# apapiu/transformer_latent_diffusion

Measured on AMD Instinct MI355X. Metric: images/sec (256px, 35-step CFG sampling), denoiser only, higher is better.
Workload: dtype bf16; 1 GPU; C1: 100M-param denoiser (d=768, L=12), 32x32x4 latents, 35 steps + CFG 6, DPM-Solver++(2M), 64 images/GPU (model batch 128); images_per_gpu=64, global_batch=64, n_iter=35, parallelism=single GPU

## Files before the change

### transformer_latent_diffusion_amd/csrc/tld_engine.hip

```cpp
#include "../../include/tld_hip.h"
#include "tld_common.h"
#include "tld_host.h"
#include "tld_refresh.h"
#include "tld_tail_fold_math.h"

#include <cmath>
#include <cstdarg>
#include <cstdio>
#include <cstring>
#include <cstdlib>
#include <map>
#include <string>
#include <unordered_map>
#include <vector>

using namespace tld;

namespace {
thread_local char g_err[512] = "";
}
namespace tld {
void set_last_error(const char* msg) { snprintf(g_err, sizeof(g_err), "%s", msg); }
thread_local uint64_t* g_path_sink = nullptr;
}
// ... 267 lines not shown
    launch_linear_f32(e->c_sin, e->ne, e->ff1_w, e->ff1_b, e->c_h1, e->d, Tn, e->ne, e->d, 1, s);
    launch_linear_f32(e->c_h1, e->d, e->ff3_w, e->ff3_b, e->c_pre, e->d, Tn, e->d, e->d, 0, s);
}

void cond_label_rows(tld_engine* e, int row0, int Tl, hipStream_t s) {
    launch_linear_f32(e->c_label, e->text, e->label_w, e->label_b, e->c_pre + (size_t)row0 * e->d, e->d, Tl,
                      e->text, e->d, 0, s);
}

int run_body(tld_engine* e, const float* x_src, int src_batch, int batch, const int* noise_row,
             const int* label_row, float* out, hipStream_t s, bool share_l0 = false, const int* src_row = nullptr) {
    const int d = e->d, M = batch * e->ntok;
    share_l0 = share_l0 && e->share_l0 && (src_row ? batch > src_batch && batch <= 2 * src_batch : batch == 2 * src_batch);
    if (int rc = debug_poison(e, s)) return rc;
    const int b0 = share_l0 ? src_batch : batch;
    resid_t* xe = share_l0 ? e->x_half : e->x;
    const bool fold1 = e->fold_ln1;
    const int ln_slots = gemm_resid_stat_slots(d);
    {
        ProfScope ps(e, KC_EMBED, s);
        EmbedParams ep{};
        ep.x = x_src; ep.conv_w = e->conv_w; ep.conv_b = e->conv_b; ep.ln1_w = e->pln1_w; ep.ln1_b = e->pln1_b;
        ep.lin_wt = e->plin_wt; ep.lin_w_hl = e->plin_w_hl; ep.lin_b = e->plin_b; ep.ln2_w = e->pln2_w; ep.ln2_b = e->pln2_b; ep.pos = e->pos;
        ep.tok = xe; ep.stats_out = fold1 ? e->ln_stats : nullptr; ep.batch = b0; ep.src_batch = src_batch; ep.C = e->cfg.n_channels;
        ep.src_row = share_l0 ? nullptr : src_row;
        ep.S = e->cfg.image_size; ep.p = e->cfg.patch_size; ep.grid = e->grid; ep.pd = e->pd; ep.d = d;
        ep.ntok = e->ntok;
        launch_embed(ep, s);
    }
    const int rdt = sizeof(resid_t) == 2 ? ST_BF16 : ST_F32;
    SNAP("tokens0", xe, rdt, s, (int64_t)b0 * e->ntok, d);
    for (int l = 0; l < e->L; ++l) {
        const Layer& Ly = e->layers[l];
        const bool half = share_l0 && l == 0;
        const int bl = half ? b0 : batch, Ml = bl * e->ntok;
        const bool fuse8 = e->fp8 && e->fp8_fused;
        SNAP(blk_name(l, "x_in"), half ? xe : e->x, rdt, s, Ml, d);
        if (fold1) SNAP(blk_name(l, "ln1"), e->ln_stats, ST_F32, s, Ml, kLnSlots, 2);
        if (!fold1) {
            ProfScope ps(e, KC_LN, s);
            if (fuse8 && layernorm_mx8_supported(d)) launch_layernorm_mx8(half ? xe : e->x, Ly.n1_w, Ly.n1_b, e->a8, e->as8, Ml, d, s);
            else { launch_layernorm_bf16(half ? xe : e->x, Ly.n1_w, Ly.n1_b, e->xn, Ml, d, s); SNAP(blk_name(l, "xn1"), e->xn, ST_BF16, s, Ml, d); }
        }
        const bool fused_qa = eng_fused_qa(e);
        if (fused_qa) {
            ProfScope ps(e, KC_GEMM_QKV, s);
            GemmParams g{};
            const bool pair = eng_qkv_pair(e, bl);
            g.A = half ? xe : e->x; g.lda = d; g.W = pair ? Ly.qkv_wp2 : Ly.qkv_wp; g.ldw = d; g.M = Ml; g.N = 3 * d; g.K = d;
            g.out_bf16 = e->att; g.ldo = d; g.ntok = e->ntok; g.d = d;
            g.ln_stats = e->ln_stats; g.ln_slots = l == 0 ? 2 : ln_slots; g.ln_c1 = pair ? Ly.qkv_c1p2 : Ly.qkv_c1p; g.ln_b1 = pair ? Ly.qkv_b1p2 : Ly.qkv_b1p;
            g.park = pair ? e->pair_park : nullptr;
            GEMM_TRY(blk_name(l, "QKV + attention"), launch_gemm(g, pair ? EPI_QKV_ATTN2 : EPI_QKV_ATTN, s));
        } else {
            ProfScope ps(e, KC_GEMM_QKV, s);
            GemmParams g{};
            g.A = e->xn; g.lda = d; g.W = Ly.qkv_w; g.ldw = d; g.M = Ml; g.N = 3 * d; g.K = d;
            g.out_bf16 = e->qk; g.ldo = 2 * d; g.vt = e->vt; g.ntok = e->ntok; g.d = d;
            if (e->fp8) {
                if (!(fuse8 && layernorm_mx8_supported(d))) launch_quant_mx8(e->xn, e->a8, e->as8, Ml, d, s);
                SNAP(blk_name(l, "a8_qkv.q"), e->a8, ST_U8, s, Ml, d); SNAP(blk_name(l, "a8_qkv.s"), e->as8, ST_MX8S, s, Ml, d / 32);
                g.f8 = 1; g.A = reinterpret_cast<const bf16*>(e->a8); g.W = reinterpret_cast<const bf16*>(Ly.qkv_w8);
                g.a_scale = e->as8; g.w_scale = Ly.qkv_s8;
            }
#ifdef TLD_RESID_BF16
            if (fold1) {
                g.A = half ? xe : e->x; g.W = Ly.qkv_wf; g.ln_stats = e->ln_stats; g.ln_slots = l == 0 ? 2 : ln_slots;
                g.ln_c1 = Ly.qkv_c1; g.ln_b1 = Ly.qkv_b1;
            }
#endif
            GEMM_TRY(blk_name(l, "QKV projection"), launch_gemm(g, fold1 ? EPI_QKV_LN : EPI_QKV, s));
            SNAP(blk_name(l, "qk"), e->qk, ST_BF16, s, Ml, 2 * d); SNAP(blk_name(l, "vt"), e->vt, ST_BF16, s, bl, d, e->ntok);
        }
        if (!fused_qa) {
            ProfScope ps(e, KC_ATTN, s);
            launch_attention(e->qk, e->vt, e->att, bl, e->ntok, e->H, s);
        }
        SNAP(blk_name(l, "att"), e->att, ST_BF16, s, Ml, d);
        const bool fuse_dw = eng_fuse_dw(e);
        const bool fold3 = e->fold_ln3;
        {
            ProfScope ps(e, KC_CROSS, s);
            CrossRowParams cp{};
            cp.x = e->x; cp.att = e->att;
            cp.x_in = half ? xe : nullptr; cp.src_batch = src_batch; cp.src_row = src_row;
            cp.wq = e->c_wq + (size_t)l * e->cond_cap * e->H * d;
            cp.bwq = e->c_bwq + (size_t)l * e->cond_cap * e->H;
            cp.v = e->c_kv + (size_t)l * e->cond_cap * 2 * d + d;
            cp.v_ld = 2 * d;
            cp.noise_row = noise_row; cp.label_row = label_row;
            cp.ln2_w = Ly.n2_w; cp.ln2_b = Ly.n2_b; cp.ln3_w = Ly.n3_w; cp.ln3_b = Ly.n3_b;
            cp.xn3 = fold3 ? nullptr : e->xn; cp.ln3_stats = fold3 ? e->row_stats : nullptr; cp.batch = batch; cp.ntok = e->ntok; cp.d = d; cp.heads = e->H;
            if (e->dbg_keep) { if (int rc = e->stages.sink(blk_name(l, "sa"), M, d, &cp.sa_out)) return rc; }
            const bool cross8 = fuse8 && cross_row_supports_ln3_stats(d);
            if (cross8) { cp.xn3_f8 = e->a8; cp.xn3_s8 = e->as8; }
            launch_cross_row(cp, s);
            if (!fold3 && !cross8) SNAP(blk_name(l, "xn3"), e->xn, ST_BF16, s, M, d);
        }
        SNAP(blk_name(l, "ca"), e->x, rdt, s, M, d);
        if (fold3) SNAP(blk_name(l, "stats"), e->row_stats, ST_F32, s, M, 2);
        if (fuse_dw) {
            ProfScope ps(e, KC_GEMM_UP, s);
            GemmParams g{};
            g.A = e->xn; g.lda = d; g.W = Ly.up_w; g.ldw = d; g.M = M; g.N = e->hid; g.K = d;
            g.out_bf16 = e->hid2; g.ldo = e->hid; g.bias = Ly.up_b; g.dw_b = Ly.dw_b_half;
            g.dw_wpk = Ly.dw_wpk;
// ... 395 lines not shown
                if (pair_form) {
                    IMG(Ly.qkv_wp2, 3 * d * d) IMG(Ly.qkv_c1p2, 3 * d) IMG(Ly.qkv_b1p2, 3 * d)
                }
            }
        }
        if (e->fp8) {
            IMG(Ly.qkv_w8, 3 * d * d) IMG(Ly.qkv_s8, 3 * d * d / 32) IMG(Ly.up_w8, hid * d) IMG(Ly.up_s8, hid * d / 32)
            IMG(Ly.down_w8, d * hid) IMG(Ly.down_s8, d * hid / 32)
        }
        if (e->fold_ln3) { IMG(Ly.up_wf, hid * d) IMG(Ly.up_c1, hid) IMG(Ly.up_b1, hid) }
        IMG(Ly.dw_w9c, 9 * hid) IMG(Ly.dw_w9c_half, 9 * hid) IMG(Ly.dw_b_half, hid) IMG(Ly.dw_wpk, 12 * hid)
    }
    if (e->fold_tail && !e->fp8) {
        const size_t n = (size_t)(2 * tail_fold_padded_rows((int)pd) * (d + hid));
        IMG(e->out_fold_hl, n) IMG(e->out_fold_b, pd)
        HIP_TRY(hipMemsetAsync(e->out_fold_hl, 0, n * sizeof(bf16), nullptr));
        R.tail_fold_hl = e->out_fold_hl; R.tail_fold_b = e->out_fold_b;
    }
#undef IMG
    {
        const size_t L = (size_t)e->L;
        std::vector<const float*> tab(4 * L);
        for (size_t l = 0; l < L; ++l) { tab[l] = e->layers[l].kv_w; tab[L + l] = e->layers[l].q_w; tab[2 * L + l] = e->layers[l].n2_w; tab[3 * L + l] = e->layers[l].n2_b; }
        const float** tabs = nullptr;
        if (int rc = dev_alloc(e, &tabs, 4 * L)) return rc;
        e->tab_kv_w = tabs; e->tab_q_w = tabs + L; e->tab_n2_w = tabs + 2 * L; e->tab_n2_b = tabs + 3 * L;
        HIP_TRY(hipMemcpy(tabs, tab.data(), 4 * L * sizeof(float*), hipMemcpyHostToDevice));
        Layer* ld = nullptr;
        if (int rc = dev_alloc(e, &ld, L)) return rc;
        HIP_TRY(hipMemcpy(ld, e->layers.data(), L * sizeof(Layer), hipMemcpyHostToDevice));
        R.layers_dev = ld;
    }
    {
        struct Flat { float* p = nullptr; ~Flat() { if (p) (void)hipFree(p); } } flat;
        HIP_TRY(hipMalloc(&flat.p, (size_t)pl.count * sizeof(float)));
        for (const ParamTensor& q : pl.tensors)
            HIP_TRY(hipMemcpy(flat.p + q.off, e->host[q.key].data.data(), (size_t)q.numel * sizeof(float), hipMemcpyHostToDevice));
        e->host.clear();
        if (int rc = launch_refresh_weights(R, flat.p, nullptr)) return rc;
        HIP_TRY(hipStreamSynchronize(nullptr));
    }

    const size_t B2 = (size_t)e->cfg.max_batch, M = B2 * e->ntok;
    if (int rc = dev_alloc(e, &e->x, M * d)) return rc;
    if (int rc = dev_alloc(e, &e->x_half, M * d)) return rc;
    if (int rc = dev_alloc(e, &e->xn, M * d)) return rc;
    if (int rc = dev_alloc(e, &e->row_stats, M + 256)) return rc;
    if (int rc = dev_alloc(e, &e->ln_stats, (M + 256) * kLnSlots)) return rc;
    if (int rc = dev_alloc(e, &e->qk, M * 2 * d)) return rc;
    if (int rc = dev_alloc(e, &e->vt, M * d)) return rc;
    if (int rc = dev_alloc(e, &e->att, M * d)) return rc;
    if (pair_form) {
        const size_t pairs = B2 * (size_t)(e->H / 2), cus = (size_t)device_cu_count();
        if (int rc = dev_alloc(e, &e->pair_park, (pairs < cus ? pairs : cus) * (size_t)kPairSlotDwords)) return rc;
    }
    if (int rc = dev_alloc(e, &e->hid1, M * hid)) return rc;
    if (e->grid == 32 && e->fuse_dwconv && hid % 256 == 0) { if (int rc = dev_alloc(e, &e->seam, M * hid / 4)) return rc; }
    if (int rc = dev_alloc(e, &e->hid2, M * hid)) return rc;
    if (e->fp8) {
        if (int rc = dev_alloc(e, &e->a8, M * hid)) return rc;
        if (int rc = dev_alloc(e, &e->as8, M * hid / 32 + 1024)) return rc;
    }
    {
        auto& P = e->poison;
        P.clear();
        P.emplace_back(e->x, M * d * sizeof(resid_t)); P.emplace_back(e->x_half, M * d * sizeof(resid_t)); P.emplace_back(e->xn, M * d * 2);
        P.emplace_back(e->row_stats, (M + 256) * sizeof(float2)); P.emplace_back(e->ln_stats, (M + 256) * kLnSlots * sizeof(float2));
        P.emplace_back(e->qk, M * 2 * d * 2); P.emplace_back(e->vt, M * d * 2); P.emplace_back(e->att, M * d * 2);
        P.emplace_back(e->hid1, M * hid * 2); P.emplace_back(e->hid2, M * hid * 2);
        if (e->seam) P.emplace_back(e->seam, M * hid / 4 * sizeof(uint32_t));
    }
    if (int rc = dev_alloc(e, &e->io_x, B2 * e->img)) return rc;
    if (int rc = dev_alloc(e, &e->io_out, B2 * e->img)) return rc;
    if (int rc = dev_alloc(e, &e->io_sigma, B2)) return rc;
    if (int rc = dev_alloc(e, &e->io_label, B2 * e->text)) return rc;
    if (int rc = dev_alloc(e, &e->xt, B2 * e->img)) return rc;
    if (int rc = dev_alloc(e, &e->x0_prev, B2 * e->img)) return rc;
    if (int rc = ensure_cond_capacity(e, 2 * (int)B2)) return rc;
    if (int rc = dev_alloc(e, &e->rows_dev, 2 * B2)) return rc;
    if (int rc = ensure_req_capacity(e, 64 * (sizeof(SamplerStepRow) + 8 * B2))) return rc;
    e->finalized = true;
    return TLD_OK;
}

int64_t tld_engine_param_count(const tld_engine* e) { return e ? e->nparam : 0; }

int tld_engine_refresh_weights(tld_engine* e, const float* flat_device, int64_t numel, void* hip_stream) {
    if (!e || !flat_device) return fail(TLD_ERR_INVALID, "null argument");
    if (!e->finalized) return fail(TLD_ERR_STATE, "tld_engine_refresh_weights: weights not finalized (the first load goes through tld_engine_load_tensor)");
    if (numel != e->nparam)
        return fail(TLD_ERR_SHAPE, "tld_engine_refresh_weights: the flat vector has %lld elements, this configuration %lld", (long long)numel, (long long)e->nparam);
    DeviceGuard dg(e->cfg.device_id);
    return launch_refresh_weights(e->refresh, flat_device, static_cast<hipStream_t>(hip_stream));
}

int tld_engine_set_debug(tld_engine* e, int32_t enable) {
    if (!e) return fail(TLD_ERR_INVALID, "null engine");
    DeviceGuard dg(e->cfg.device_id);
    if (enable) {
        if (!e->finalized) return fail(TLD_ERR_STATE, "tld_engine_set_debug: weights not finalized");
        e->debug = true;
        if (int rc = reserve_snapshots(e)) { (void)hipDeviceSynchronize(); e->stages.free_all(); e->debug = false; return rc; }
    } else {
        (void)hipDeviceSynchronize();
        e->stages.free_all();
        e->debug = false; e->dbg_keep = false;
    }
// ... 504 lines not shown
```

### transformer_latent_diffusion_amd/csrc/tld_gemm.hip

```cpp
#include "../../include/tld_hip.h"
#include "tld_common.h"
#include "tld_attn_core.h"
#include <cstdlib>
#include <cstring>
#include <type_traits>

#ifdef TLD_DBG_EPI
#define TLD_EPI_BIT(b) ((p.dbg_epi & (b)) != 0)
#else
#define TLD_EPI_BIT(b) false
#endif

namespace tld {

namespace {

typedef const __attribute__((address_space(1))) void* gptr_t;
typedef __attribute__((address_space(3))) void* lptr_t;

__device__ __forceinline__ bf16x8 read_frag(const char* lds_tile, int row, int kchunk) {
    const int off = row * 128 + ((kchunk ^ ((row >> 1) & 7)) << 4);
    return *reinterpret_cast<const bf16x8*>(lds_tile + off);
}

template <int BN>
struct G256 {
    static constexpr int BM = 256, BK = 64;
    static constexpr int WN = (BN >= 256) ? 4 : 2, WMc = 8 / WN;
    static constexpr int WROWS = BM / WMc;
    static constexpr int WCOLS = BN / WN;
    static constexpr int TM = WROWS / 32, TN = WCOLS / 32;
    static constexpr int A_BYTES = BM * BK * 2, B_BYTES = BN * BK * 2;
    static constexpr int A_PIECES = BM / 8 / 8, B_PIECES = BN / 8 / 8;
};

template <int N> __device__ __forceinline__ void wait_vmcnt() {
    if constexpr (N == 0) asm volatile("s_waitcnt vmcnt(0)" ::: "memory");
    else if constexpr (N == 3) asm volatile("s_waitcnt vmcnt(3)" ::: "memory");
    else if constexpr (N == 4) asm volatile("s_waitcnt vmcnt(4)" ::: "memory");
    else if constexpr (N == 6) asm volatile("s_waitcnt vmcnt(6)" ::: "memory");
    else if constexpr (N == 7) asm volatile("s_waitcnt vmcnt(7)" ::: "memory");
    else if constexpr (N == 8) asm volatile("s_waitcnt vmcnt(8)" ::: "memory");
    else static_assert(N < 0, "unsupported vmcnt");
}

template <int BN>
struct G256P : G256<BN> {
    static constexpr int STAGES = 2;
    static constexpr int STAGE_BYTES = G256<BN>::A_BYTES + G256<BN>::B_BYTES;
    static constexpr int LDS_BYTES = 2 * STAGE_BYTES;
    static constexpr int LN_RAW = LDS_BYTES, LN_ST = LN_RAW + 256 * 8 * kLnSlots, LN_CB = LN_ST + 256 * 8, QKVLN_LDS = LN_CB + 2048;
    static constexpr int IMG2_PITCH = 1024, IMG2_BYTES = 128 * IMG2_PITCH;
    static constexpr int ZROW_OFF = IMG2_BYTES, ZROW_BYTES = 16 * IMG2_PITCH;
    static constexpr int ROWSTAT2_OFF = ZROW_OFF + ZROW_BYTES;
    static constexpr int CB2_OFF = ROWSTAT2_OFF + 256 * 8;
    static constexpr int UPDW2_LDS = CB2_OFF + 2048;
    static constexpr int PLAINRS_OFF = LDS_BYTES;
    static constexpr int PLAINCB_OFF = PLAINRS_OFF + 256 * 8;
    static constexpr int PLAINLN_LDS = PLAINCB_OFF + 2048;
    static constexpr int SCRATCH = 4608;
    static constexpr int AT_K = STAGE_BYTES, AT_V = AT_K + 256 * 128, AT_Q = AT_V + 64 * kAttnVPitch, ATTN_LDS = AT_Q + 256 * 128;
    static constexpr int P2_RAW = 0, P2_ST = P2_RAW + 256 * 8 * kLnSlots, P2_CB = P2_ST + 256 * 8;
    static constexpr int P2_K = P2_CB + 2 * 384 * 4 + 3072, P2_V = P2_K + 256 * 128, P2_Q = P2_V + 64 * kAttnVPitch, PAIR_LDS_END = P2_Q + 256 * 128;
};

template <int BN, int EPI, bool F8 = false, bool CONV = false, bool RING = false, bool TN = false>
__global__ __launch_bounds__(512) void gemm256p_kernel(GemmParams p, int nblocks) {
    using G = G256P<BN>;
    static_assert(!RING || BN == 256, "the half-tile ring exists for 256 x 256 tiles (bf16, and since round 6 MX-fp8)");
    static_assert(!TN || (BN == 256 && EPI == EPI_F32 && !F8 && !CONV && !RING), "transposed operands: fp32 output, 256 x 256 tiles, two-stage loop");
    using frag_t = std::conditional_t<F8, i32x8, bf16x8>;
    constexpr int ESZ = F8 ? 1 : 2;
    constexpr int SC_OFF = G::LDS_BYTES;
    static_assert(!F8 || (EPI == EPI_F32 || EPI == EPI_QKV || EPI == EPI_BIAS_BF16 || EPI == EPI_BIAS_RESID), "fp8 epilogues");
    static_assert(!CONV || (!F8 && (EPI == EPI_F32 || EPI == EPI_BIAS_BF16 || EPI == EPI_BIAS_RESID)), "conv mode");
    constexpr bool PLAIN_CB = EPI == EPI_BIAS_BF16 && BN != 384 && !F8 && !CONV;
    constexpr bool IS_QKV = EPI == EPI_QKV || EPI == EPI_QKV_LN, LN = EPI == EPI_QKV_LN || EPI == EPI_QKV_ATTN;
    constexpr bool UPDW = EPI == EPI_UP_DWCONV2 || EPI == EPI_UP_DWCONV32;
    static_assert(EPI != EPI_QKV_ATTN || (BN == 192 && !F8 && !CONV && !RING), "the fused attention epilogue is written for 256 x 192 tiles");
    static_assert(EPI != EPI_QKV_ATTN || G::ATTN_LDS <= 160 * 1024, "LDS");
    constexpr bool PAIR = EPI == EPI_QKV_ATTN2;
    static_assert(!PAIR || (BN == 384 && !F8 && !CONV && !RING && !TN), "the two-head attention epilogue is written for 256 x 384 tiles");
    static_assert(!PAIR || G::PAIR_LDS_END <= G::LDS_BYTES, "LDS");
    constexpr bool COLD = UPDW || PAIR;
    static_assert(8 * G::SCRATCH <= G::STAGE_BYTES, "epilogue scratch must fit in one stage");
    extern __shared__ __attribute__((aligned(16))) char smem[];
    const int lane = threadIdx.x & 63;
    const int wid = __builtin_amdgcn_readfirstlane(threadIdx.x >> 6);
    const int wm = wid / G::WN, wn = wid % G::WN;
    const int l31 = lane & 31, hi = lane >> 5;

    const int ntn = (p.N + BN - 1) / BN;
    const int ntm = (p.M + G::BM - 1) / G::BM;
    constexpr bool KSPLIT_OK = EPI == EPI_F32 && !F8 && !CONV && !RING && !TN;
    const int nsplit = (KSPLIT_OK && p.ksplit > 1) ? p.ksplit : 1;
    const int ntiles = ntm * ntn * nsplit;
    int kb_dec = 0;
    const int bid = blockIdx.x;
    const int xcd = bid & 7, lidx = bid >> 3;
    const int per_xcd_blocks = (nblocks + 7 - xcd) / 8;
    const int G2 = p.xcd_ngroups > 1 ? p.xcd_ngroups : 1;
    const int xn = xcd % G2, xm = xcd / G2, XM = 8 / G2;
    const int gcols = ntn / G2;
    const int r0 = (int)((long)ntm * xm / XM), r1 = (int)((long)ntm * (xm + 1) / XM);
    const int q = ntiles >> 3, rr = ntiles & 7;
    const int xbase = xcd < rr ? xcd * (q + 1) : rr * (q + 1) + (xcd - rr) * q;
    const int xcount = G2 > 1 ? (r1 - r0) * gcols : q + (xcd < rr ? 1 : 0);
    int my_tiles = lidx < xcount ? (xcount - lidx + per_xcd_blocks - 1) / per_xcd_blocks : 0;
    constexpr bool HT_OK = RING && !CONV && (EPI == EPI_F32 || EPI == EPI_QKV || EPI == EPI_QKV_LN || EPI == EPI_BIAS_BF16);
    const int ht_q = xcount / per_xcd_blocks, ht_R = xcount - ht_q * per_xcd_blocks;
    const bool ht = HT_OK && p.half_tail && G2 == 1 && ht_R > 0 && 2 * ht_R <= per_xcd_blocks;
    const int ht_qa = lidx >= ht_R ? 1 : 0;
    if (ht) my_tiles = ht_q + (lidx < 2 * ht_R ? 1 : 0);
    auto item_tile = [&](int i) {
        if (ht && i == ht_q) return ht_q * per_xcd_blocks + (lidx < ht_R ? lidx : lidx - ht_R);
        return lidx + i * per_xcd_blocks;
    };
    auto tile_coords = [&](int i, int& m0, int& n0) {
        const int t = item_tile(i);
        if (G2 > 1) {
            const int tm = t / gcols;
            m0 = (r0 + tm) * G::BM;
            n0 = (xn * gcols + (t - tm * gcols)) * BN;
        } else {
            int tile = xbase + t;
            if constexpr (KSPLIT_OK) {
                if (nsplit > 1) {
                    const int sp = tile / (ntm * ntn);
                    tile -= sp * (ntm * ntn);
                    kb_dec = sp * p.K * 2;
                }
            }
            const int tm = tile / ntn;
            m0 = tm * G::BM;
            n0 = (tile - tm * ntn) * BN;
        }
// ... 355 lines not shown
                    __builtin_amdgcn_global_load_lds((gptr_t)src, (lptr_t)(smem + G::P2_CB + (wid & 1) * 1536 + (wid >> 1) * 1024), 16, 0, 0);
                }
            }
            if constexpr (EPI == EPI_BIAS_BF16) {
                if (BN != 384 && p.row_stats && wid < 2) {
                    int r0s = m0 + wid * 128 + lane * 2;
                    r0s = r0s + 1 < p.M ? r0s : (p.M >= 2 ? p.M - 2 : 0);
                    const char* src = reinterpret_cast<const char*>(p.row_stats + r0s);
                    __builtin_amdgcn_global_load_lds((gptr_t)src, (lptr_t)(smem + G::PLAINRS_OFF + wid * 1024), 16, 0, 0);
                }
                if constexpr (PLAIN_CB) {
                    if (wid == 3 || (wid == 2 && p.row_stats)) {
                        int col = n0 + lane * 4;
                        col = col < p.N ? col : 0;
                        const float* src = (wid == 2 ? p.ln_c1 : p.bias) + col;
                        __builtin_amdgcn_global_load_lds((gptr_t)src, (lptr_t)(smem + G::PLAINCB_OFF + (wid - 2) * 1024), 16, 0, 0);
                    }
                }
            }
            if constexpr (UPDW) {
                constexpr int RS_OFF = G::ROWSTAT2_OFF;
                if (p.row_stats && wid < 2) {
                    const char* src = reinterpret_cast<const char*>(p.row_stats + m0) + wid * 1024 + lane * 16;
                    __builtin_amdgcn_global_load_lds((gptr_t)src, (lptr_t)(smem + RS_OFF + wid * 1024), 16, 0, 0);
                }
                if (wid == 3 || (wid == 2 && p.row_stats)) {
                    const float* src = (wid == 2 ? p.ln_c1 : p.bias) + n0 + lane * 4;
                    __builtin_amdgcn_global_load_lds((gptr_t)src, (lptr_t)(smem + G::CB2_OFF + (wid - 2) * 1024), 16, 0, 0);
                }
            }
        };
        auto kloop = [&](auto swp) {
            constexpr bool SW = decltype(swp)::value;
            auto mma = [&](const frag_t (&a)[G::TM], const frag_t (&b)[G::TN], auto slice) {
                constexpr int S2 = decltype(slice)::value * 2;
#pragma unroll
                for (int i = 0; i < G::TM; ++i)
#pragma unroll
                    for (int j = 0; j < G::TN; ++j) {
                        if constexpr (F8) {
                            if constexpr (SW) acc[i][j] = __builtin_amdgcn_mfma_scale_f32_32x32x64_f8f6f4(b[j], a[i], acc[i][j], 0, 0, S2, scb[j], S2, sca[i]);
                            else acc[i][j] = __builtin_amdgcn_mfma_scale_f32_32x32x64_f8f6f4(a[i], b[j], acc[i][j], 0, 0, S2, sca[i], S2, scb[j]);
                        } else {
                            if constexpr (SW) acc[i][j] = __builtin_amdgcn_mfma_f32_32x32x16_bf16(b[j], a[i], acc[i][j], 0, 0, 0);
                            else acc[i][j] = __builtin_amdgcn_mfma_f32_32x32x16_bf16(a[i], b[j], acc[i][j], 0, 0, 0);
                        }
                    }
            };
            constexpr int NP = G::A_PIECES + G::B_PIECES;
            {
            const int grp = wid >> 2;
            wait_vmcnt<0>();
            __builtin_amdgcn_s_barrier();
            if (grp) __builtin_amdgcn_s_barrier();
            for (int k = 0; k < nkt; ++k, ++g) {
                if (k == (PAIR ? nkt - 1 : nkt > 1 ? 1 : 0)) aux_dma();
                const char* st = smem + (g & 1) * G::STAGE_BYTES;
                char* nst = smem + ((g + 1) & 1) * G::STAGE_BYTES;
                const bool more = (k + 1 < nkt) || (has_next && !COLD);
                const int pkb = (k + 1 < nkt) ? (KSPLIT_OK ? kb0 : 0) + (k + 1) * G::BK * 2 : (KSPLIT_OK ? kbn : 0);
                if constexpr (CONV) {
                    if (k + 1 < nkt) {
                        if (++ccb == kpt) { ccb = 0; ++ctap; conv_tap(ctap); }
                    } else { ccb = 0; ctap = 0; }
                    conv_akb = ccb * (G::BK * 2);
                }
                if (k + 1 == nkt && more) set_offsets(m0n, n0n);
                constexpr int NI = F8 ? 2 : 4;
                constexpr int NDMA = (NI == 4) ? 2 : 1;
#pragma unroll
                for (int h = 0; h < NI; ++h) {
                    load_frags(st, h, a0, b0);
                    if constexpr (F8) {
                        if (h == 0) {
                            const char* sc = smem + SC_OFF + (g & 1) * 2048;
#pragma unroll
                            for (int i = 0; i < G::TM; ++i) sca[i] = *reinterpret_cast<const int*>(sc + (wm * G::WROWS + i * 32 + l31) * 4) >> (8 * hi);
#pragma unroll
                            for (int j = 0; j < G::TN; ++j) scb[j] = *reinterpret_cast<const int*>(sc + 1024 + (wn * G::WCOLS + j * 32 + l31) * 4) >> (8 * hi);
                        }
                    }
                    if (h < NDMA && more) {
                        constexpr int PER = (NP + NDMA - 1) / NDMA;
#pragma unroll
                        for (int q2 = 0; q2 < NP; ++q2) {
                            if (q2 < h * PER || q2 >= (h + 1) * PER) continue;
                            dma_piece(q2, pkb, nst);
                        }
                        if (h == 0) {
                            if (k + 1 < nkt) dma_scales(m0, n0, k + 1, (g + 1) & 1);
                            else dma_scales(m0n, n0n, 0, (g + 1) & 1);
                        }
                    }
                    if (h == NI - 1) wait_vmcnt<0>();
                    if (h == NI - 1) asm volatile("s_waitcnt lgkmcnt(0)" ::: "memory");
                    __builtin_amdgcn_sched_barrier(0);
                    __builtin_amdgcn_s_barrier();
                    __builtin_amdgcn_sched_barrier(0);
                    __builtin_amdgcn_s_setprio(1);
                    if constexpr (F8) {
                        if (h == 0) mma(a0, b0, std::integral_constant<int, 0>{}); else mma(a0, b0, std::integral_constant<int, 1>{});
                    } else {
                        mma(a0, b0, std::integral_constant<int, 0>{});
                    }
                    __builtin_amdgcn_s_setprio(0);
                    if (h == NI - 1) wait_vmcnt<0>();
// ... 113 lines not shown
                        auto cat = [](const piece_t& lo, const piece_t& hi4) {
                            return i32x8{(int)lo[0], (int)lo[1], (int)lo[2], (int)lo[3], (int)hi4[0], (int)hi4[1], (int)hi4[2], (int)hi4[3]};
                        };
                        __builtin_amdgcn_s_setprio(1);
#pragma unroll
                        for (int sl = 0; sl < 2; ++sl) {
                            const i32x8 bo = qb ? cat(fb1[2 * sl], fb1[2 * sl + 1]) : cat(fb0[2 * sl], fb0[2 * sl + 1]);
#pragma unroll
                            for (int ii = 0; ii < 2; ++ii) {
                                const i32x8 ao = cat(fa[ii][2 * sl], fa[ii][2 * sl + 1]);
                                const int sa = ii ? sa1 : sa0;
                                if (sl == 0) {
                                    if constexpr (SW) acc[qa * 2 + ii][qb] = __builtin_amdgcn_mfma_scale_f32_32x32x64_f8f6f4(bo, ao, acc[qa * 2 + ii][qb], 0, 0, 0, sb, 0, sa);
                                    else acc[qa * 2 + ii][qb] = __builtin_amdgcn_mfma_scale_f32_32x32x64_f8f6f4(ao, bo, acc[qa * 2 + ii][qb], 0, 0, 0, sa, 0, sb);
                                } else {
                                    if constexpr (SW) acc[qa * 2 + ii][qb] = __builtin_amdgcn_mfma_scale_f32_32x32x64_f8f6f4(bo, ao, acc[qa * 2 + ii][qb], 0, 0, 2, sb, 2, sa);
                                    else acc[qa * 2 + ii][qb] = __builtin_amdgcn_mfma_scale_f32_32x32x64_f8f6f4(ao, bo, acc[qa * 2 + ii][qb], 0, 0, 2, sa, 2, sb);
                                }
                            }
                        }
                        __builtin_amdgcn_s_setprio(0);
                    } else {
                    __builtin_amdgcn_s_setprio(1);
#pragma unroll
                    for (int ks = 0; ks < 4; ++ks)
#pragma unroll
                        for (int ii = 0; ii < 2; ++ii) {
                            const piece_t& bf = qb ? fb1[ks] : fb0[ks];
                            if constexpr (SW) acc[qa * 2 + ii][qb] = __builtin_amdgcn_mfma_f32_32x32x16_bf16(bf, fa[ii][ks], acc[qa * 2 + ii][qb], 0, 0, 0);
                            else acc[qa * 2 + ii][qb] = __builtin_amdgcn_mfma_f32_32x32x16_bf16(fa[ii][ks], bf, acc[qa * 2 + ii][qb], 0, 0, 0);
                        }
                    __builtin_amdgcn_s_setprio(0);
                    }
                    }
                    __builtin_amdgcn_sched_barrier(0);
                    __builtin_amdgcn_s_barrier();
                    __builtin_amdgcn_sched_barrier(0);
                };
                phase(std::integral_constant<int, 1>{}); phase(std::integral_constant<int, 2>{});
                phase(std::integral_constant<int, 3>{}); phase(std::integral_constant<int, 4>{});
                phase(std::integral_constant<int, 5>{}); phase(std::integral_constant<int, 6>{});
                phase(std::integral_constant<int, 7>{}); phase(std::integral_constant<int, 8>{});
            };
            for (int j = 0; j + 1 < nj; ++j) iter(j, std::false_type{});
            iter(nj - 1, std::true_type{});
            if (xt) wait_vmcnt<0>();
            if (!grp) __builtin_amdgcn_s_barrier();
            g += nk;
            }
        };
        if constexpr (RING) {
            if constexpr (swapped) kloop_ring(std::true_type{}); else kloop_ring(std::false_type{});
        } else {
            if constexpr (swapped) kloop(std::true_type{}); else kloop(std::false_type{});
        }

        const int row0 = m0 + wm * G::WROWS;
        const int col0 = n0 + wn * G::WCOLS;
        auto gn_combine = [&](const float2* red) {
            if constexpr (CONV) {
                asm volatile("s_waitcnt lgkmcnt(0)" ::: "memory");
                __builtin_amdgcn_s_barrier();
                const int tid = wid * 64 + lane;
                const int qpg = p.gn_cpg >> 2;
                if (tid < BN / p.gn_cpg) {
                    float a = 0.f, a2 = 0.f;
                    for (int w2 = 0; w2 < G::WMc; ++w2)
                        for (int k2 = 0; k2 < qpg; ++k2) { const float2 t = red[w2 * (BN / 4) + tid * qpg + k2]; a += t.x; a2 += t.y; }
                    const int bb = m0 / p.gn_hw;
                    const int chunk = (m0 - bb * p.gn_hw) >> 8, nchunk = p.gn_hw >> 8;
                    p.gn_partial[((size_t)bb * nchunk + chunk) * p.gn_groups + n0 / p.gn_cpg + tid] = make_float2(a, a2);
                }
            }
        };
        if constexpr (EPI == EPI_F32) {
#pragma unroll
            for (int i = 0; i < G::TM; ++i)
#pragma unroll
                for (int j = 0; j < G::TN; ++j) {
                    const int col = col0 + j * 32 + l31;
                    if (col >= p.N || (hmode && (i >> 1) != ht_qa)) continue;
#pragma unroll
                    for (int r = 0; r < 16; ++r) {
                        const int row = row0 + i * 32 + 4 * hi + (r & 3) + 8 * (r >> 2);
                        if (row < p.M) p.c_f32[(KSPLIT_OK && nsplit > 1 ? (size_t)(kb0 / (p.K * 2)) * p.M * p.ldc : (size_t)0) + (size_t)row * p.ldc + col] = acc[i][j][r];
                    }
                }
        } else {
            __builtin_amdgcn_s_barrier();
            char* ws = RING ? smem + 4 * HT + wid * G::SCRATCH : smem + ((g - 1) & 1) * G::STAGE_BYTES + wid * G::SCRATCH;
            if constexpr (UPDW) {
                static_assert(BN == 256, "fused depthwise epilogue is written for 256-column tiles");
                char* H = smem;
                {
                    if (it == 0) {
                        *reinterpret_cast<u32x4*>(smem + G::ZROW_OFF + threadIdx.x * 16) = u32x4{0u, 0u, 0u, 0u};
                        *reinterpret_cast<u32x4*>(smem + G::ZROW_OFF + 8192 + threadIdx.x * 16) = u32x4{0u, 0u, 0u, 0u};
                    }
                }
                const bool ln3 = p.row_stats != nullptr;
                float cst[G::TN], bst[G::TN];
#pragma unroll
                for (int j = 0; j < G::TN; ++j) {
                    const int cl = wn * 64 + j * 32 + l31;
                    bst[j] = *reinterpret_cast<const float*>(smem + G::CB2_OFF + 1024 + cl * 4);
                    cst[j] = ln3 ? *reinterpret_cast<const float*>(smem + G::CB2_OFF + cl * 4) : 0.f;
                }
// ... 365 lines not shown
#else
                    const float inv = attn256_wave(Kimg, Vimg, qf, o, e_l31, e_hi);
#endif
                    char* T = Qimg + wid * 4096;
                    bf16* dst0 = p.out_bf16 + (size_t)(m0 + q0) * p.ldo + (n0 / BN) * 64;
#pragma unroll
                    for (int half = 0; half < 2; ++half) {
                        if ((e_l31 >> 4) == half) {
#pragma unroll
                            for (int ct = 0; ct < 2; ++ct)
#pragma unroll
                                for (int rq = 0; rq < 4; ++rq) {
                                    bf16x4 pk;
#pragma unroll
                                    for (int e2 = 0; e2 < 4; ++e2) pk[e2] = (bf16)(o[ct][rq * 4 + e2] * inv);
                                    *reinterpret_cast<bf16x4*>(T + (e_l31 & 15) * 144 + ct * 64 + rq * 16 + e_hi * 8) = pk;
                                }
                        }
                        __builtin_amdgcn_fence(__ATOMIC_RELEASE, "wavefront");
#pragma unroll
                        for (int it2 = 0; it2 < 2; ++it2) {
                            const int r = it2 * 8 + (e_lane >> 3), c16 = e_lane & 7;
                            const u32x4 w = *reinterpret_cast<const u32x4*>(T + r * 144 + c16 * 16);
                            __builtin_nontemporal_store(w, reinterpret_cast<u32x4*>(dst0 + (size_t)(half * 16 + r) * p.ldo + c16 * 8));
                        }
                        __builtin_amdgcn_fence(__ATOMIC_ACQUIRE, "wavefront");
                    }
                }
            } else if constexpr (PAIR) {
                int e_lane = lane, e_l31 = l31, e_hi = hi;
                asm volatile("" : "+v"(e_lane), "+v"(e_l31), "+v"(e_hi));
                const int tid = wid * 64 + e_lane;
                {
                    const int s0 = (tid & 1) * 4;
                    const float4* raw = reinterpret_cast<const float4*>(smem + G::P2_RAW + (tid >> 1) * 64 + s0 * 8);
                    float su = 0.f, sq = 0.f;
#pragma unroll
                    for (int q2 = 0; q2 < 2; ++q2)
                        if (s0 + 2 * q2 < p.ln_slots) {
                            const float4 v = raw[q2];
                            su += v.x + v.z; sq += v.y + v.w;
                        }
                    su = dpp_add<0xB1>(su); sq = dpp_add<0xB1>(sq);
                    int kdim = p.K;
                    asm volatile("" : "+s"(kdim));
                    const float inv_k = 1.0f / (float)kdim;
                    const float mu = su * inv_k;
                    const float var = fmaxf(fmaf(sq, inv_k, -mu * mu), 0.f);
                    if (!(tid & 1))
                        reinterpret_cast<float2*>(smem + G::P2_ST)[tid >> 1] = make_float2(mu, __builtin_amdgcn_rsqf(var + kLnEps));
                    asm volatile("s_waitcnt lgkmcnt(0)" ::: "memory");
                    __builtin_amdgcn_s_barrier();
                }
                u32x4* slot = reinterpret_cast<u32x4*>(p.park) + (size_t)blockIdx.x * (kPairSlotDwords / 4) + tid;
                bf16x8 pk[G::TM][G::TN];
                {
                    float rs[G::TM], nm[G::TM];
#pragma unroll
                    for (int i = 0; i < G::TM; ++i) {
                        const float2 st = reinterpret_cast<const float2*>(smem + G::P2_ST)[wm * G::WROWS + i * 32 + e_l31];
                        rs[i] = st.y; nm[i] = -st.y * st.x;
                    }
#pragma unroll
                    for (int j = 0; j < G::TN; ++j) {
#pragma unroll
                        for (int rq = 0; rq < 4; ++rq) {
                            const int cl = wn * G::WCOLS + j * 32 + 8 * rq + 4 * e_hi;
                            const float4 c4 = *reinterpret_cast<const float4*>(smem + G::P2_CB + cl * 4);
                            const float4 b4 = *reinterpret_cast<const float4*>(smem + G::P2_CB + 1536 + cl * 4);
#pragma unroll
                            for (int i = 0; i < G::TM; ++i) {
                                acc[i][j][rq * 4 + 0] = fmaf(rs[i], acc[i][j][rq * 4 + 0], fmaf(nm[i], c4.x, b4.x));
                                acc[i][j][rq * 4 + 1] = fmaf(rs[i], acc[i][j][rq * 4 + 1], fmaf(nm[i], c4.y, b4.y));
                                acc[i][j][rq * 4 + 2] = fmaf(rs[i], acc[i][j][rq * 4 + 2], fmaf(nm[i], c4.z, b4.z));
                                acc[i][j][rq * 4 + 3] = fmaf(rs[i], acc[i][j][rq * 4 + 3], fmaf(nm[i], c4.w, b4.w));
                            }
                        }
#pragma unroll
                        for (int i = 0; i < G::TM; ++i) {
                            bf16x8 b;
#pragma unroll
                            for (int e2 = 0; e2 < 8; ++e2) b[e2] = (bf16)acc[i][j][8 + e2];
                            slot[(j * G::TM + i) * 512] = __builtin_bit_cast(u32x4, b);
                        }
                    }
#pragma unroll
                    for (int j = 0; j < G::TN; ++j)
#pragma unroll
                        for (int i = 0; i < G::TM; ++i)
#pragma unroll
                            for (int e2 = 0; e2 < 8; ++e2) pk[i][j][e2] = (bf16)acc[i][j][e2];
                }
                char* Kimg = smem + G::P2_K;
                char* Vimg = smem + G::P2_V;
                char* Qimg = smem + G::P2_Q;
                auto head = [&](int side) {
#pragma unroll
                    for (int j = 0; j < G::TN; ++j) {
#pragma unroll
                        for (int i = 0; i < G::TM; ++i) {
                            const int row = wm * G::WROWS + i * 32 + e_l31;
#pragma unroll
                            for (int rq = 0; rq < 2; ++rq) {
                                const bf16x4 q4 = {pk[i][j][rq * 4 + 0], pk[i][j][rq * 4 + 1], pk[i][j][rq * 4 + 2], pk[i][j][rq * 4 + 3]};
                                const int f = wn * 16 + 8 * rq + 4 * e_hi;
                                if (j < 2) {
                                    char* img = j == 0 ? Qimg : Kimg;
                                    *reinterpret_cast<bf16x4*>(img + row * 128 + ((((f >> 3) ^ ((row >> 1) & 7)) << 4) | ((f & 7) << 1))) = q4;
                                } else {
#pragma unroll
                                    for (int e2 = 0; e2 < 4; ++e2)
                                        *reinterpret_cast<bf16*>(Vimg + (f + e2) * kAttnVPitch + row * 2) = q4[e2];
                                }
                            }
                        }
                    }
                    asm volatile("s_waitcnt lgkmcnt(0)" ::: "memory");
                    __builtin_amdgcn_s_barrier();
                    const int q0 = wid * 32;
                    bf16x8 qf[4];
                    {
                        const int row = q0 + e_l31;
#pragma unroll
                        for (int ks = 0; ks < 4; ++ks)
                            qf[ks] = *reinterpret_cast<const bf16x8*>(Qimg + row * 128 + (((ks * 2 + e_hi) ^ ((row >> 1) & 7)) << 4));
                    }
                    f32x16 o[2];
                    const float inv = attn256_wave(Kimg, Vimg, qf, o, e_l31, e_hi);
                    char* T = Qimg + wid * 4096;
                    bf16* dst0 = p.out_bf16 + (size_t)(m0 + q0) * p.ldo + ((n0 / BN) * 2 + side) * 64;
#pragma unroll
                    for (int half = 0; half < 2; ++half) {
                        if ((e_l31 >> 4) == half) {
#pragma unroll
                            for (int ct = 0; ct < 2; ++ct)
#pragma unroll
                                for (int rq = 0; rq < 4; ++rq) {
                                    bf16x4 o4;
#pragma unroll
                                    for (int e2 = 0; e2 < 4; ++e2) o4[e2] = (bf16)(o[ct][rq * 4 + e2] * inv);
                                    *reinterpret_cast<bf16x4*>(T + (e_l31 & 15) * 144 + ct * 64 + rq * 16 + e_hi * 8) = o4;
                                }
                        }
                        __builtin_amdgcn_fence(__ATOMIC_RELEASE, "wavefront");
#pragma unroll
                        for (int it2 = 0; it2 < 2; ++it2) {
                            const int r = it2 * 8 + (e_lane >> 3), c16 = e_lane & 7;
                            const u32x4 w = *reinterpret_cast<const u32x4*>(T + r * 144 + c16 * 16);
                            __builtin_nontemporal_store(w, reinterpret_cast<u32x4*>(dst0 + (size_t)(half * 16 + r) * p.ldo + c16 * 8));
                        }
                        __builtin_amdgcn_fence(__ATOMIC_ACQUIRE, "wavefront");
                    }
                };
                head(0);
                wait_vmcnt<0>();
#pragma unroll
                for (int j = 0; j < G::TN; ++j)
#pragma unroll
                    for (int i = 0; i < G::TM; ++i) pk[i][j] = __builtin_bit_cast(bf16x8, slot[(j * G::TM + i) * 512]);
                __builtin_amdgcn_s_barrier();
                head(1);
                __builtin_amdgcn_s_barrier();
                if (has_next) issue(m0n, n0n, g);
            } else if constexpr (EPI == EPI_BIAS_BF16 && G::WCOLS == 96) {
                constexpr int P = 64 + 16;
                int e_lane = lane, e_l31 = l31, e_hi = hi;
                asm volatile("" : "+v"(e_lane), "+v"(e_l31), "+v"(e_hi));
#pragma unroll
                for (int i = 0; i < G::TM; ++i)
#pragma unroll
                    for (int j = 0; j < G::TN; ++j) {
#pragma unroll
                        for (int rq = 0; rq < 4; ++rq) {
                            const int cl = 8 * rq + 4 * e_hi;
                            const int cg = col0 + j * 32 + cl < p.N ? col0 + j * 32 + cl : 0;
                            const float4 bv = *reinterpret_cast<const float4*>(p.bias + cg);
                            bf16x4 pk;
                            pk[0] = (bf16)(acc[i][j][rq * 4 + 0] + bv.x); pk[1] = (bf16)(acc[i][j][rq * 4 + 1] + bv.y);
                            pk[2] = (bf16)(acc[i][j][rq * 4 + 2] + bv.z); pk[3] = (bf16)(acc[i][j][rq * 4 + 3] + bv.w);
                            *reinterpret_cast<bf16x4*>(ws + e_l31 * P + cl * 2) = pk;
                        }
#pragma unroll
                        for (int itr = 0; itr < 2; ++itr) {
                            const int idx = itr * 64 + e_lane;
                            const int rl = idx >> 2, ch = idx & 3;
                            const u32x4 v = *reinterpret_cast<const u32x4*>(ws + rl * P + ch * 16);
                            const int row = row0 + i * 32 + rl, col = col0 + j * 32 + ch * 8;
                            if (row < p.M && col < p.N) TLD_STORE(reinterpret_cast<u32x4*>(p.out_bf16 + (size_t)row * p.ldo + col), v);
                        }
                    }
            } else if constexpr (G::WCOLS == 64) {
                int e_lane = lane, e_l31 = l31, e_hi = hi;
                asm volatile("" : "+v"(e_lane), "+v"(e_l31), "+v"(e_hi));
                if constexpr (LN) {
                    {
                        const int tid = wid * 64 + e_lane;
                        const int s0 = (tid & 1) * 4;
                        const float4* raw = reinterpret_cast<const float4*>(smem + G::LN_RAW + (tid >> 1) * 64 + s0 * 8);
                        float su = 0.f, sq = 0.f;
#pragma unroll
                        for (int q2 = 0; q2 < 2; ++q2)
                            if (s0 + 2 * q2 < p.ln_slots) {
                                const float4 v = raw[q2];
                                su += v.x + v.z; sq += v.y + v.w;
                            }
                        su = dpp_add<0xB1>(su); sq = dpp_add<0xB1>(sq);
                        const float inv_k = 1.0f / (float)p.K;
                        const float mu = su * inv_k;
                        const float var = fmaxf(fmaf(sq, inv_k, -mu * mu), 0.f);
                        if (!(tid & 1))
                            reinterpret_cast<float2*>(smem + G::LN_ST)[tid >> 1] = make_float2(mu, __builtin_amdgcn_rsqf(var + kLnEps));
                        asm volatile("s_waitcnt lgkmcnt(0)" ::: "memory");
                        __builtin_amdgcn_s_barrier();
                    }
                    float rs[G::TM], nm[G::TM];
// ... 310 lines not shown
```

### transformer_latent_diffusion_amd/csrc/tld_gemm_params.h

```cpp
#pragma once
#include <stdint.h>
#ifndef __HIP__
struct float2;
#endif

namespace tld {

typedef __bf16 bf16;

#ifdef TLD_RESID_FP32
typedef float resid_t;
#else
#define TLD_RESID_BF16 1
typedef __bf16 resid_t;
#endif

constexpr int kLnSlots = 8;

enum GemmEpilogue {
    EPI_F32 = 0,
    EPI_QKV = 1,
    EPI_BIAS_BF16 = 2,
    EPI_BIAS_RESID = 3,
    EPI_QKV_LN = 5,
    EPI_UP_DWCONV32 = 4,
    EPI_UP_DWCONV2 = 6,
    EPI_QKV_ATTN = 7,
    EPI_QKV_ATTN2 = 9,
};

struct GemmParams {
    const bf16* A; int lda;
    const bf16* W; int ldw;
    int M, N, K;
    float* c_f32; int ldc;
    bf16* out_bf16; int ldo;
    bf16* vt;
    int ntok, d;
    const float* bias;
    const float* dw_b;
    uint32_t* dw_seam;
    const uint32_t* dw_wpk;
    resid_t* resid; int ldr;
    float2* stats_out;
    const float2* ln_stats;
    int ln_slots;
    const float* ln_b1;
    const float2* row_stats;
    const float* ln_c1;
    int f8;
    const uint8_t* a_scale;
    const uint8_t* w_scale;
    int w_batch_rows;
    unsigned w_batch_stride_bytes;
    int conv, cv_h, cv_w, cv_up, cv_cin;
    unsigned cv_data_off;
    float2* gn_partial;
    int gn_groups, gn_cpg, gn_hw;
    int ksplit;
    int xcd_ngroups;
    int tn_ktotal;
    int half_tail;
    int dbg_epi;
    int cv_down;
    uint32_t* park;
};

constexpr int kPairSlotDwords = 512 * 48;

}
```

Before: 317.5 images/s.

## Park half of the pair-attention QKV fragments in spare LDS instead of global memory

In the two-head fused QKV+attention epilogue, the second-half accumulator fragments were all parked in a per-block global scratch slot and reloaded after the first head. Six of the twelve entries now go into unused LDS regions around the pair layout, and the global slot shrinks to the other six. The global reloads are issued inside head 0, right after its output store, so they overlap with the remaining stores. The attention output staging also switches to a swizzled 32-row tile written in one pass instead of two 16-row halves. A compile-gated timestamp trace is added for profiling. The risk is more LDS pressure and possible layout conflicts, which the new static asserts are meant to catch.

```diff
diff --git a/transformer_latent_diffusion_amd/csrc/tld_engine.hip b/transformer_latent_diffusion_amd/csrc/tld_engine.hip
--- a/transformer_latent_diffusion_amd/csrc/tld_engine.hip
+++ b/transformer_latent_diffusion_amd/csrc/tld_engine.hip
@@ -343,6 +343,26 @@
             g.ln_stats = e->ln_stats; g.ln_slots = l == 0 ? 2 : ln_slots; g.ln_c1 = pair ? Ly.qkv_c1p2 : Ly.qkv_c1p; g.ln_b1 = pair ? Ly.qkv_b1p2 : Ly.qkv_b1p;
             g.park = pair ? e->pair_park : nullptr;
             GEMM_TRY(blk_name(l, "QKV + attention"), launch_gemm(g, pair ? EPI_QKV_ATTN2 : EPI_QKV_ATTN, s));
+#ifdef TLD_GEMM_TRACE_BUILD
+            if (pair) {
+                static int launches = 0;
+                static const char* path = getenv("TLD_GEMM_TRACE");
+                static const int at = getenv("TLD_GEMM_TRACE_LAUNCH") ? atoi(getenv("TLD_GEMM_TRACE_LAUNCH")) : 200;
+                if (path && ++launches == at) {
+                    std::vector<unsigned long long> st(kPairTraceDwords / 2);
+                    HIP_TRY(hipStreamSynchronize(s));
+                    HIP_TRY(hipMemcpy(st.data(), e->pair_park, (size_t)kPairTraceDwords * 4, hipMemcpyDeviceToHost));
+                    if (FILE* f = fopen(path, "w")) {
+                        for (int r = 0; r < 24; ++r) {
+                            fprintf(f, "tile %d wave %d", r / 8, r % 8);
+                            for (int c = 0; c < 13; ++c) fprintf(f, " %llu", st[r * 16 + c]);
+                            fprintf(f, "\n");
+                        }
+                        fclose(f);
+                    }
+                }
+            }
+#endif
         } else {
             ProfScope ps(e, KC_GEMM_QKV, s);
             GemmParams g{};
@@ -844,7 +864,7 @@
     if (int rc = dev_alloc(e, &e->att, M * d)) return rc;
     if (pair_form) {
         const size_t pairs = B2 * (size_t)(e->H / 2), cus = (size_t)device_cu_count();
-        if (int rc = dev_alloc(e, &e->pair_park, (pairs < cus ? pairs : cus) * (size_t)kPairSlotDwords)) return rc;
+        if (int rc = dev_alloc(e, &e->pair_park, (pairs < cus ? pairs : cus) * (size_t)kPairSlotDwords + kPairTraceDwords)) return rc;
     }
     if (int rc = dev_alloc(e, &e->hid1, M * hid)) return rc;
     if (e->grid == 32 && e->fuse_dwconv && hid % 256 == 0) { if (int rc = dev_alloc(e, &e->seam, M * hid / 4)) return rc; }
diff --git a/transformer_latent_diffusion_amd/csrc/tld_gemm.hip b/transformer_latent_diffusion_amd/csrc/tld_gemm.hip
--- a/transformer_latent_diffusion_amd/csrc/tld_gemm.hip
+++ b/transformer_latent_diffusion_amd/csrc/tld_gemm.hip
@@ -43,6 +43,13 @@
     else if constexpr (N == 8) asm volatile("s_waitcnt vmcnt(8)" ::: "memory");
     else static_assert(N < 0, "unsupported vmcnt");
 }
+
+#ifdef TLD_GEMM_TRACE_BUILD
+#define TLD_PAIR_STAMP(slot_) do { if constexpr (PAIR) { if (blockIdx.x == 0 && it < 3 && lane == 0) \
+    reinterpret_cast<unsigned long long*>(p.park)[(it * 8 + wid) * 16 + (slot_)] = __builtin_amdgcn_s_memtime(); } } while (0)
+#else
+#define TLD_PAIR_STAMP(slot_) do { } while (0)
+#endif
 
 template <int BN>
 struct G256P : G256<BN> {
@@ -62,6 +69,9 @@
     static constexpr int AT_K = STAGE_BYTES, AT_V = AT_K + 256 * 128, AT_Q = AT_V + 64 * kAttnVPitch, ATTN_LDS = AT_Q + 256 * 128;
     static constexpr int P2_RAW = 0, P2_ST = P2_RAW + 256 * 8 * kLnSlots, P2_CB = P2_ST + 256 * 8;
     static constexpr int P2_K = P2_CB + 2 * 384 * 4 + 3072, P2_V = P2_K + 256 * 128, P2_Q = P2_V + 64 * kAttnVPitch, PAIR_LDS_END = P2_Q + 256 * 128;
+    static constexpr int PARK_ENTRY = 512 * 16, PARK_LO = P2_RAW, PARK_LO_N = (P2_ST - P2_RAW) / PARK_ENTRY, PARK_HI = PAIR_LDS_END, PARK_HI_N = 4;
+    static constexpr int PARK_LDS = PARK_LO_N + PARK_HI_N, PARK_LO_END = PARK_LO + PARK_LO_N * PARK_ENTRY, PARK_HI_END = PARK_HI + PARK_HI_N * PARK_ENTRY;
+    static constexpr int park_lds_off(int e) { return e < PARK_LO_N ? PARK_LO + e * PARK_ENTRY : PARK_HI + (e - PARK_LO_N) * PARK_ENTRY; }
 };
 
 template <int BN, int EPI, bool F8 = false, bool CONV = false, bool RING = false, bool TN = false>
@@ -82,6 +92,11 @@
     constexpr bool PAIR = EPI == EPI_QKV_ATTN2;
     static_assert(!PAIR || (BN == 384 && !F8 && !CONV && !RING && !TN), "the two-head attention epilogue is written for 256 x 384 tiles");
     static_assert(!PAIR || G::PAIR_LDS_END <= G::LDS_BYTES, "LDS");
+    static_assert(!PAIR || (G::LDS_BYTES == 160 * 1024 && G::PARK_HI_END <= 160 * 1024 && G::PARK_LO >= 0), "parked entries: inside the CU's 160 KiB");
+    static_assert(!PAIR || (G::PARK_LO_END <= G::P2_ST && G::PARK_HI >= G::PAIR_LDS_END), "parked entries: disjoint from (mean, rstd), c1 | b1 and the K, V^T, Q images");
+    static_assert(!PAIR || (G::P2_ST < G::P2_CB && G::P2_CB < G::P2_K && G::P2_K < G::P2_V && G::P2_V < G::P2_Q && G::P2_Q < G::PAIR_LDS_END), "pair layout order");
+    static_assert(!PAIR || (G::PARK_LDS == 6 && G::PARK_LDS * G::PARK_ENTRY + kPairSlotDwords * 4 == 12 * G::PARK_ENTRY), "6 entries in LDS, 6 in the slot");
+    static_assert(!PAIR || (G::PARK_LO % 16 == 0 && G::PARK_HI % 16 == 0), "16-byte lane accesses");
     constexpr bool COLD = UPDW || PAIR;
     static_assert(8 * G::SCRATCH <= G::STAGE_BYTES, "epilogue scratch must fit in one stage");
     extern __shared__ __attribute__((aligned(16))) char smem[];
@@ -543,6 +558,7 @@
             const int grp = wid >> 2;
             wait_vmcnt<0>();
             __builtin_amdgcn_s_barrier();
+            TLD_PAIR_STAMP(1);
             if (grp) __builtin_amdgcn_s_barrier();
             for (int k = 0; k < nkt; ++k, ++g) {
                 if (k == (PAIR ? nkt - 1 : nkt > 1 ? 1 : 0)) aux_dma();
@@ -762,7 +778,9 @@
         if constexpr (RING) {
             if constexpr (swapped) kloop_ring(std::true_type{}); else kloop_ring(std::false_type{});
         } else {
+            TLD_PAIR_STAMP(0);
             if constexpr (swapped) kloop(std::true_type{}); else kloop(std::false_type{});
+            TLD_PAIR_STAMP(2);
         }
 
         const int row0 = m0 + wm * G::WROWS;
@@ -1234,7 +1252,14 @@
                     asm volatile("s_waitcnt lgkmcnt(0)" ::: "memory");
                     __builtin_amdgcn_s_barrier();
                 }
-                u32x4* slot = reinterpret_cast<u32x4*>(p.park) + (size_t)blockIdx.x * (kPairSlotDwords / 4) + tid;
+                auto park_slot = [&](int e) {
+                    char* b = reinterpret_cast<char*>(p.park + kPairTraceDwords) + (size_t)blockIdx.x * (kPairSlotDwords * 4) + (e - G::PARK_LDS) * G::PARK_ENTRY;
+                    asm volatile("" : "+s"(b));
+                    unsigned vo = (unsigned)tid * 16;
+                    asm volatile("" : "+v"(vo));
+                    return (__attribute__((address_space(1))) u32x4*)(b + vo);
+                };
+                auto park_lds = [&](int e) { return reinterpret_cast<u32x4*>(smem + G::park_lds_off(e) + tid * 16); };
                 bf16x8 pk[G::TM][G::TN];
                 {
                     float rs[G::TM], nm[G::TM];
@@ -1263,7 +1288,9 @@
                             bf16x8 b;
 #pragma unroll
                             for (int e2 = 0; e2 < 8; ++e2) b[e2] = (bf16)acc[i][j][8 + e2];
-                            slot[(j * G::TM + i) * 512] = __builtin_bit_cast(u32x4, b);
+                            const int e = j * G::TM + i;
+                            if (e < G::PARK_LDS) *park_lds(e) = __builtin_bit_cast(u32x4, b);
+                            else *park_slot(e) = __builtin_bit_cast(u32x4, b);
                         }
                     }
 #pragma unroll
@@ -1273,10 +1300,12 @@
 #pragma unroll
                             for (int e2 = 0; e2 < 8; ++e2) pk[i][j][e2] = (bf16)acc[i][j][e2];
                 }
+                TLD_PAIR_STAMP(3);
                 char* Kimg = smem + G::P2_K;
                 char* Vimg = smem + G::P2_V;
                 char* Qimg = smem + G::P2_Q;
-                auto head = [&](int side) {
+                auto head = [&](auto sidec) {
+                    constexpr int side = decltype(sidec)::value;
 #pragma unroll
                     for (int j = 0; j < G::TN; ++j) {
 #pragma unroll
@@ -1299,6 +1328,7 @@
                     }
                     asm volatile("s_waitcnt lgkmcnt(0)" ::: "memory");
                     __builtin_amdgcn_s_barrier();
+                    TLD_PAIR_STAMP(4 + side * 5);
                     const int q0 = wid * 32;
                     bf16x8 qf[4];
                     {
@@ -1309,40 +1339,42 @@
                     }
                     f32x16 o[2];
                     const float inv = attn256_wave(Kimg, Vimg, qf, o, e_l31, e_hi);
+                    TLD_PAIR_STAMP(5 + side * 5);
                     char* T = Qimg + wid * 4096;
                     bf16* dst0 = p.out_bf16 + (size_t)(m0 + q0) * p.ldo + ((n0 / BN) * 2 + side) * 64;
 #pragma unroll
-                    for (int half = 0; half < 2; ++half) {
-                        if ((e_l31 >> 4) == half) {
-#pragma unroll
-                            for (int ct = 0; ct < 2; ++ct)
-#pragma unroll
-                                for (int rq = 0; rq < 4; ++rq) {
-                                    bf16x4 o4;
-#pragma unroll
-                                    for (int e2 = 0; e2 < 4; ++e2) o4[e2] = (bf16)(o[ct][rq * 4 + e2] * inv);
-                                    *reinterpret_cast<bf16x4*>(T + (e_l31 & 15) * 144 + ct * 64 + rq * 16 + e_hi * 8) = o4;
-                                }
-                        }
-                        __builtin_amdgcn_fence(__ATOMIC_RELEASE, "wavefront");
-#pragma unroll
-                        for (int it2 = 0; it2 < 2; ++it2) {
-                            const int r = it2 * 8 + (e_lane >> 3), c16 = e_lane & 7;
-                            const u32x4 w = *reinterpret_cast<const u32x4*>(T + r * 144 + c16 * 16);
-                            __builtin_nontemporal_store(w, reinterpret_cast<u32x4*>(dst0 + (size_t)(half * 16 + r) * p.ldo + c16 * 8));
-                        }
-                        __builtin_amdgcn_fence(__ATOMIC_ACQUIRE, "wavefront");
-                    }
+                    for (int ct = 0; ct < 2; ++ct)
+#pragma unroll
+                        for (int rq = 0; rq < 4; ++rq) {
+                            bf16x4 o4;
+#pragma unroll
+                            for (int e2 = 0; e2 < 4; ++e2) o4[e2] = (bf16)(o[ct][rq * 4 + e2] * inv);
+                            *reinterpret_cast<bf16x4*>(T + e_l31 * 128 + (((ct * 4 + rq) ^ (e_l31 & 7)) << 4) + e_hi * 8) = o4;
+                        }
+                    __builtin_amdgcn_fence(__ATOMIC_RELEASE, "wavefront");
+                    if constexpr (side == 0) {
+#pragma unroll
+                        for (int e = G::PARK_LDS; e < G::TM * G::TN; ++e) pk[e % G::TM][e / G::TM] = __builtin_bit_cast(bf16x8, *park_slot(e));
+                    }
+#pragma unroll
+                    for (int it2 = 0; it2 < 4; ++it2) {
+                        const int r = it2 * 8 + (e_lane >> 3), c16 = e_lane & 7;
+                        const u32x4 w = *reinterpret_cast<const u32x4*>(T + r * 128 + ((c16 ^ (r & 7)) << 4));
+                        __builtin_nontemporal_store(w, reinterpret_cast<u32x4*>(dst0 + (size_t)r * p.ldo + c16 * 8));
+                    }
+                    __builtin_amdgcn_fence(__ATOMIC_ACQUIRE, "wavefront");
                 };
-                head(0);
-                wait_vmcnt<0>();
-#pragma unroll
-                for (int j = 0; j < G::TN; ++j)
-#pragma unroll
-                    for (int i = 0; i < G::TM; ++i) pk[i][j] = __builtin_bit_cast(bf16x8, slot[(j * G::TM + i) * 512]);
+                head(std::integral_constant<int, 0>{});
+                TLD_PAIR_STAMP(6);
+                TLD_PAIR_STAMP(7);
+#pragma unroll
+                for (int e = 0; e < G::PARK_LDS; ++e) pk[e % G::TM][e / G::TM] = __builtin_bit_cast(bf16x8, *park_lds(e));
                 __builtin_amdgcn_s_barrier();
-                head(1);
+                TLD_PAIR_STAMP(8);
+                head(std::integral_constant<int, 1>{});
+                TLD_PAIR_STAMP(11);
                 __builtin_amdgcn_s_barrier();
+                TLD_PAIR_STAMP(12);
                 if (has_next) issue(m0n, n0n, g);
             } else if constexpr (EPI == EPI_BIAS_BF16 && G::WCOLS == 96) {
                 constexpr int P = 64 + 16;
diff --git a/transformer_latent_diffusion_amd/csrc/tld_gemm_params.h b/transformer_latent_diffusion_amd/csrc/tld_gemm_params.h
--- a/transformer_latent_diffusion_amd/csrc/tld_gemm_params.h
+++ b/transformer_latent_diffusion_amd/csrc/tld_gemm_params.h
@@ -66,6 +66,11 @@
     uint32_t* park;
 };
 
-constexpr int kPairSlotDwords = 512 * 48;
+constexpr int kPairSlotDwords = 512 * 24;
+#ifdef TLD_GEMM_TRACE_BUILD
+constexpr int kPairTraceDwords = 1024;
+#else
+constexpr int kPairTraceDwords = 0;
+#endif
 
 }
```

Result: no change. 322.3 images/s (median of 6 runs) (+1.5%).
